# vitasoftAI/ImageRetrievalResearch

Hardware: AMD Instinct MI355X
Metric: images/sec embed + queries/sec top-k@100k-gallery, EffNet-B3a 224^2 (higher is better)
Workload: dtype bf16

## Files before the change

imageretrievalresearch_amd/csrc/rank.hip:

```cpp
#include "rank_common.h"
#include "../../include/mi355_retrieval.h"

#include <limits.h>
#include <stdlib.h>
#include <math.h>

namespace mi355 {

template <bool WRITE_ROWS>
__global__ __launch_bounds__(256) void k_row_norm(const float* __restrict__ in, float* __restrict__ out,
                                                  float* __restrict__ inv, i64 rows, int dim, float eps,
                                                  int vec) {
    const int lane = threadIdx.x & 63;
    const i64 row = (i64)blockIdx.x * 4 + (threadIdx.x >> 6);
    if (row >= rows) return;
    const float* x = in + row * dim;
    const float r = row_inv_norm(x, dim, eps, vec, lane);
    if (inv != nullptr && lane == 0) inv[row] = r;
    if (WRITE_ROWS) {
        float* y = out + row * dim;
        if (vec) {
            const f32x4* x4 = reinterpret_cast<const f32x4*>(x);
            f32x4* y4 = reinterpret_cast<f32x4*>(y);
            for (int i = lane; i < dim / 4; i += 64) {
// ... 128 lines not shown
        for (int i = 0; i < A_LOADS; ++i)
            *reinterpret_cast<f32x4*>(a + (r0 + RPP * i) * RK_LD + c4 * 4) = ra[i];
#pragma unroll
        for (int i = 0; i < B_LOADS; ++i)
            *reinterpret_cast<f32x4*>(b + (r0 + RPP * i) * RK_LD + c4 * 4) = rb[i];
    };

    const int nt = (D + RK_BK - 1) / RK_BK;
    load_tile(0);
    store_tile(0);
    __syncthreads();

    const int lr = lane & 31;
    const int lk = (lane >> 5) * 4;
    for (int t = 0; t < nt; ++t) {
        const int buf = t & 1;
        if (t + 1 < nt) load_tile((t + 1) * RK_BK);
        const float* a = As + buf * BM * RK_LD + (wm * MT * 32 + lr) * RK_LD + lk;
        const float* b = Bs + buf * RK_BN * RK_LD + (wn * 64 + lr) * RK_LD + lk;
#pragma unroll
        for (int t8 = 0; t8 < RK_BK / 8; ++t8) {
            f32x4 af[MT], bfr[2];
#pragma unroll
            for (int i = 0; i < MT; ++i) af[i] = *reinterpret_cast<const f32x4*>(a + i * 32 * RK_LD + t8 * 8);
#pragma unroll
            for (int j = 0; j < 2; ++j) bfr[j] = *reinterpret_cast<const f32x4*>(b + j * 32 * RK_LD + t8 * 8);
#pragma unroll
            for (int e = 0; e < 4; ++e)
#pragma unroll
                for (int i = 0; i < MT; ++i)
#pragma unroll
                    for (int j = 0; j < 2; ++j)
                        acc[i][j] = __builtin_amdgcn_mfma_f32_32x32x2f32(af[i][e], bfr[j][e], acc[i][j], 0, 0, 0);
        }
        if (t + 1 < nt) store_tile(buf ^ 1);
        __syncthreads();
    }

    epi.tile(acc, smem, ginv, TileCtx{Q, G, ntx, n0, m0});
}
template <int MT, int RK_BK, bool VEC, int FK>
__global__ __launch_bounds__(256) void k_cos_gemm(const float* __restrict__ Qn, const float* __restrict__ Gal,
                                                  const float* __restrict__ ginv, int Q, i64 G, int D, int x0, int ntx,
                                                  int xtiles, int ny, PlainEpi<FK> epi) {
    cos_gemm_f32_tile<MT, RK_BK, VEC>(Qn, Gal, ginv, Q, G, D, x0, ntx, xtiles, ny, epi);
}
template <int MT, int RK_BK, bool VEC, class Epi>
__global__ __launch_bounds__(256) void k_cos_gemm_epi(const float* __restrict__ Qn, const float* __restrict__ Gal,
                                                      const float* __restrict__ ginv, int Q, i64 G, int D, int x0, int ntx,
                                                      int xtiles, int ny, Epi epi) {
    cos_gemm_f32_tile<MT, RK_BK, VEC>(Qn, Gal, ginv, Q, G, D, x0, ntx, xtiles, ny, epi);
}

template <int MT, class Epi>
__device__ __forceinline__ void cos_gemm_split_tile(const bf16_t* __restrict__ Qs, const float* __restrict__ Gal,
                                                    const float* __restrict__ ginv, int Q, i64 G, int D, int x0, int ntx,
                                                    int n_steps, const float* __restrict__ zeros, int xtiles, int ny,
                                                    const Epi& epi) {
    constexpr int BM = 64 * MT;
    constexpr int BK = 16;
    constexpr int A_STAGE = (BM / 32) * 3 * 512;
    constexpr int A_PIECES = (BM / 32) * 3;
    constexpr int B_STAGE = RK_BN * BK;
    extern __shared__ __attribute__((aligned(16))) float smem[];
    bf16_t* As = reinterpret_cast<bf16_t*>(smem);
    constexpr int A_RING = MT == 1 ? 3 : 2;
    float* Bs = smem + (A_RING * A_STAGE * 2) / 4;

    const int tid = threadIdx.x, lane = tid & 63, wave = tid >> 6;
    const int wm = wave >> 1, wn = wave & 1;
    int bx, by;
    rank_tile_of((int)blockIdx.x, xtiles, ny, bx, by);
    const i64 n0 = (i64)(bx + x0) * RK_BN;
    const int m0 = by * BM;
    const int swave = __builtin_amdgcn_readfirstlane(wave);

    const float* b_row[2];
    int b_k[2];
    bool b_ok[2];
#pragma unroll
    for (int i = 0; i < 2; ++i) {
        const int r = (swave * 2 + i) * 16 + (lane >> 2);
        const int c = (lane & 3) ^ ((r >> 2) & 3);
        b_ok[i] = n0 + r < G;
        b_row[i] = Gal + (b_ok[i] ? (n0 + r) * D : 0);
        b_k[i] = c * 4;
    }
    auto dma_b = [&](int stage, int k0) {
#pragma unroll
        for (int i = 0; i < 2; ++i) {
            const bool ok = b_ok[i] && k0 + b_k[i] < D;
            glds16(reinterpret_cast<const bf16_t*>(ok ? b_row[i] + k0 + b_k[i] : zeros),
                   reinterpret_cast<bf16_t*>(Bs + stage * B_STAGE + (swave * 2 + i) * 256));
        }
    };
    const bf16_t* a_src = Qs + (size_t)(m0 / 32) * n_steps * 3 * 512 + lane * 8;
    const bf16_t* a_piece[(A_PIECES + 3) / 4];
#pragma unroll
    for (int i = 0; i < (A_PIECES + 3) / 4; ++i) {
        const int piece = (swave + 4 * i) % A_PIECES;
        a_piece[i] = a_src + ((size_t)((piece / 3) * n_steps) * 3 + piece % 3) * 512;
    }
    auto dma_a = [&](int buf, int t) {
#pragma unroll
        for (int i = 0; i < (A_PIECES + 3) / 4; ++i) {
            const int piece = swave + 4 * i;
            if (A_PIECES % 4 == 0 || i < A_PIECES / 4 || swave < A_PIECES % 4)
                glds16(a_piece[i] + (size_t)t * 3 * 512, As + buf * A_STAGE + piece * 512);
        }
    };

    f32x16 acc[MT][2];
#pragma unroll
    for (int i = 0; i < MT; ++i)
#pragma unroll
        for (int j = 0; j < 2; ++j)
#pragma unroll
            for (int e = 0; e < 16; ++e) acc[i][j][e] = 0.f;

    const int lr = lane & 31;
    int b_off[2][2];
#pragma unroll
    for (int j = 0; j < 2; ++j) {
        const int r = wn * 64 + j * 32 + lr, sw = (r >> 2) & 3, c0 = (lane >> 5) * 2;
        b_off[j][0] = r * BK + ((c0 ^ sw) << 2);
        b_off[j][1] = r * BK + (((c0 + 1) ^ sw) << 2);
    }
    auto compute = [&](int abuf, int bstage) {
        const bf16_t* a = As + abuf * A_STAGE + (wm * MT * 3) * 512 + lane * 8;
        const float* b = Bs + bstage * B_STAGE;
        bf16x8 af[MT][3];
        u32x4 bh[2], bm[2], bl[2];
        f32x4 v0[2], v1[2];
#pragma unroll
        for (int j = 0; j < 2; ++j) {
            v0[j] = *reinterpret_cast<const f32x4*>(b + b_off[j][0]);
            v1[j] = *reinterpret_cast<const f32x4*>(b + b_off[j][1]);
        }
#pragma unroll
        for (int i = 0; i < MT; ++i)
#pragma unroll
            for (int p = 0; p < 3; ++p) af[i][p] = *reinterpret_cast<const bf16x8*>(a + (i * 3 + p) * 512);
        split3(v0[0], v1[0], bh[0], bm[0], bl[0]);
        auto products = [&](int j) {
            const bf16x8 gh = *reinterpret_cast<const bf16x8*>(&bh[j]);
            const bf16x8 gm = *reinterpret_cast<const bf16x8*>(&bm[j]);
            const bf16x8 gl = *reinterpret_cast<const bf16x8*>(&bl[j]);
#pragma unroll
            for (int i = 0; i < MT; ++i) {
                acc[i][j] = __builtin_amdgcn_mfma_f32_32x32x16_bf16(af[i][2], gh, acc[i][j], 0, 0, 0);
                acc[i][j] = __builtin_amdgcn_mfma_f32_32x32x16_bf16(af[i][0], gl, acc[i][j], 0, 0, 0);
                acc[i][j] = __builtin_amdgcn_mfma_f32_32x32x16_bf16(af[i][1], gm, acc[i][j], 0, 0, 0);
                acc[i][j] = __builtin_amdgcn_mfma_f32_32x32x16_bf16(af[i][1], gh, acc[i][j], 0, 0, 0);
                acc[i][j] = __builtin_amdgcn_mfma_f32_32x32x16_bf16(af[i][0], gm, acc[i][j], 0, 0, 0);
                acc[i][j] = __builtin_amdgcn_mfma_f32_32x32x16_bf16(af[i][0], gh, acc[i][j], 0, 0, 0);
            }
        };
        split3(v0[1], v1[1], bh[1], bm[1], bl[1]);
        products(0);
#pragma unroll
        for (int g = 0; g < 6 * MT; ++g) {
            __builtin_amdgcn_sched_group_barrier(0x008, 1, 0);
            __builtin_amdgcn_sched_group_barrier(0x002, 4, 0);
        }
        products(1);
    };

    dma_a(0, 0);
    if (A_RING == 3 && n_steps > 1) dma_a(1, 1);
    dma_b(0, 0);
    dma_b(1, BK);
    __syncthreads();

    int bs_cur = 0, bs_far = 2;
    for (int t = 0; t < n_steps; ++t) {
        if constexpr (A_RING == 2) {
            if (t + 1 < n_steps) dma_a((t & 1) ^ 1, t + 1);
        } else {
            if (t + 2 < n_steps) dma_a(bs_far, t + 2);
        }
        __builtin_amdgcn_sched_barrier(0);
        dma_b(bs_far, (t + 2) * BK);
        __builtin_amdgcn_sched_barrier(0);
        compute(A_RING == 2 ? (t & 1) : bs_cur, bs_cur);
        if constexpr (A_RING == 2) {
            asm volatile("s_waitcnt vmcnt(2)" ::: "memory");
        } else {
            if (t + 2 >= n_steps) asm volatile("s_waitcnt vmcnt(2)" ::: "memory");
            else if (swave < A_PIECES % 4) asm volatile("s_waitcnt vmcnt(4)" ::: "memory");
            else asm volatile("s_waitcnt vmcnt(3)" ::: "memory");
        }
        asm volatile("s_waitcnt lgkmcnt(0)" ::: "memory");
        __builtin_amdgcn_s_barrier();
        asm volatile("" ::: "memory");
        bs_cur = bs_cur == 2 ? 0 : bs_cur + 1;
        bs_far = bs_far == 2 ? 0 : bs_far + 1;
    }
    __syncthreads();
    epi.tile(acc, smem, ginv, TileCtx{Q, G, ntx, n0, m0});
}
template <int MT, int FK>
__global__ __launch_bounds__(256, 3) void k_cos_gemm_split(const bf16_t* __restrict__ Qs, const float* __restrict__ Gal,
                                                           const float* __restrict__ ginv, int Q, i64 G, int D, int x0, int ntx,
                                                           int n_steps, const float* __restrict__ zeros, int xtiles, int ny,
                                                           PlainEpi<FK> epi) {
    cos_gemm_split_tile<MT>(Qs, Gal, ginv, Q, G, D, x0, ntx, n_steps, zeros, xtiles, ny, epi);
}
template <int MT, class Epi>
__global__ __launch_bounds__(256, 3) void k_cos_gemm_split_epi(const bf16_t* __restrict__ Qs, const float* __restrict__ Gal,
                                                               const float* __restrict__ ginv, int Q, i64 G, int D, int x0,
                                                               int ntx, int n_steps, const float* __restrict__ zeros, int xtiles,
                                                               int ny, Epi epi) {
    cos_gemm_split_tile<MT>(Qs, Gal, ginv, Q, G, D, x0, ntx, n_steps, zeros, xtiles, ny, epi);
}

template <int MT, int FK>
__global__ __launch_bounds__(256, 2) void k_cos_gemm_pre(const bf16_t* __restrict__ Qs, const bf16_t* __restrict__ Gs, int Q,
                                                         i64 G, int x0, int ntx, int n_steps, int xtiles, int ny,
                                                         SelectEpi<FK, false> epi) {
    constexpr int BM = 64 * MT;
    constexpr int A_PIECES = (BM / 32) * 3;
    constexpr int A_STAGE = A_PIECES * 512;
    constexpr int B_PIECES = (RK_BN / 32) * 3;
    constexpr int B_STAGE = B_PIECES * 512;
    constexpr int A_RING = MT == 1 ? 3 : 2;
    extern __shared__ __attribute__((aligned(16))) float smem[];
    bf16_t* As = reinterpret_cast<bf16_t*>(smem);
    bf16_t* Bs = As + A_RING * A_STAGE;

    const int tid = threadIdx.x, lane = tid & 63, wave = tid >> 6;
    const int wm = wave >> 1, wn = wave & 1;
    int bx, by;
    rank_tile_of((int)blockIdx.x, xtiles, ny, bx, by);
    const i64 n0 = (i64)(bx + x0) * RK_BN;
    const int m0 = by * BM;
    const int swave = __builtin_amdgcn_readfirstlane(wave);

    const bf16_t* a_src = Qs + (size_t)(m0 / 32) * n_steps * 3 * 512 + lane * 8;
    const bf16_t* b_src = Gs + (size_t)(n0 / 32) * n_steps * 3 * 512 + lane * 8;
    const bf16_t* a_piece[(A_PIECES + 3) / 4];
    const bf16_t* b_piece[3];
#pragma unroll
    for (int i = 0; i < (A_PIECES + 3) / 4; ++i) {
        const int piece = (swave + 4 * i) % A_PIECES;
        a_piece[i] = a_src + ((size_t)((piece / 3) * n_steps) * 3 + piece % 3) * 512;
    }
#pragma unroll
    for (int i = 0; i < 3; ++i) {
        const int piece = swave + 4 * i;
        b_piece[i] = b_src + ((size_t)((piece / 3) * n_steps) * 3 + piece % 3) * 512;
    }
    auto dma_a = [&](int buf, int t) {
#pragma unroll
        for (int i = 0; i < (A_PIECES + 3) / 4; ++i) {
            const int piece = swave + 4 * i;
            if (A_PIECES % 4 == 0 || i < A_PIECES / 4 || swave < A_PIECES % 4)
                glds16(a_piece[i] + (size_t)t * 3 * 512, As + buf * A_STAGE + piece * 512);
        }
    };
    auto dma_b = [&](int stage, int t) {
        const int tt = t < n_steps ? t : n_steps - 1;
#pragma unroll
        for (int i = 0; i < 3; ++i) glds16(b_piece[i] + (size_t)tt * 3 * 512, Bs + stage * B_STAGE + (swave + 4 * i) * 512);
    };

    f32x16 acc[MT][2];
// ... 481 lines not shown
}

int kernel_slots(const void* fn, size_t lds, int* cache, int* slots_out) {
    int dev = 0;
    MI355_CHECK_HIP(hipGetDevice(&dev));
    MI355_REQUIRE(dev >= 0 && dev < MI355_MAX_DEVICES, "rank: device ordinal %d out of range", dev);
    if (!cache[dev]) {
        MI355_CHECK_HIP(hipFuncSetAttribute(fn, hipFuncAttributeMaxDynamicSharedMemorySize, (int)lds));
        int per_cu = 0, cus = 0;
        MI355_CHECK_HIP(hipOccupancyMaxActiveBlocksPerMultiprocessor(&per_cu, fn, 256, lds));
        MI355_CHECK_HIP(hipDeviceGetAttribute(&cus, hipDeviceAttributeMultiprocessorCount, dev));
        cache[dev] = (per_cu > 0 ? per_cu : 1) * (cus > 0 ? cus : 1);
    }
    *slots_out = cache[dev];
    return OK;
}

int whole_round_tiles(int ntx, int ny, int slots) {
    if ((long)ntx * ny > slots && ((long)ntx * ny) % slots != 0) return (int)(((long)ntx * ny / slots) * slots / ny);
    return ntx;
}

static thread_local int g_round_slots = 0;
static thread_local int g_last_tiles[5] = {0, 0, 0, 0, 0};
int round_slots(int device_slots) { return g_round_slots > 0 ? g_round_slots : device_slots; }
void set_last_tiles(int slots, int ny, int main_tiles, int tail_tiles, int tail_ny) {
    g_last_tiles[0] = slots; g_last_tiles[1] = ny; g_last_tiles[2] = main_tiles; g_last_tiles[3] = tail_tiles;
    g_last_tiles[4] = tail_ny;
}

template <bool VEC>
struct F32Gemm {
    template <int MT> static constexpr int BK = MT == 2 ? 16 : 32;
    template <int MT> static constexpr size_t stage_bytes() { return (size_t)2 * (64 * MT + RK_BN) * (BK<MT> + 4) * sizeof(float); }
    template <int MT, class Epi> static constexpr auto kernel() {
        if constexpr (plain_fk<Epi> >= 0) return &k_cos_gemm<MT, BK<MT>, VEC, plain_fk<Epi>>;
        else return &k_cos_gemm_epi<MT, BK<MT>, VEC, Epi>;
    }
    template <int MT, class Epi>
    static void launch(dim3 grid, size_t lds, hipStream_t st, const TileArgs& a, const Epi& epi, int x0, int ntx, int xtiles, int ny) {
        hipLaunchKernelGGL((kernel<MT, Epi>()), grid, dim3(256), lds, st, (const float*)a.qry, (const float*)a.gal, a.ginv, a.Q, a.G,
                           a.D, x0, ntx, xtiles, ny, epi);
    }
};

struct SplitGemm {
    template <int MT> static constexpr size_t stage_bytes() {
        return (size_t)(MT == 1 ? 3 : 2) * (64 * MT / 32) * 3 * 1024 + (size_t)3 * RK_BN * 16 * sizeof(float);
    }
    template <int MT, class Epi> static constexpr auto kernel() {
        if constexpr (plain_fk<Epi> >= 0) return &k_cos_gemm_split<MT, plain_fk<Epi>>;
        else return &k_cos_gemm_split_epi<MT, Epi>;
    }
    template <int MT, class Epi>
    static void launch(dim3 grid, size_t lds, hipStream_t st, const TileArgs& a, const Epi& epi, int x0, int ntx, int xtiles, int ny) {
        const bf16_t* qs = (const bf16_t*)a.qry;
        const int n_steps = cdiv(a.D, 16);
        const float* zeros = reinterpret_cast<const float*>(qs + (size_t)cdiv(a.Q, 128) * 4 * n_steps * 3 * 512);
        hipLaunchKernelGGL((kernel<MT, Epi>()), grid, dim3(256), lds, st, qs, (const float*)a.gal, a.ginv, a.Q, a.G, a.D, x0, ntx,
                           n_steps, zeros, xtiles, ny, epi);
    }
};

struct PreparedGemm {
    template <int MT> static constexpr size_t stage_bytes() {
        return (size_t)(MT == 1 ? 3 : 2) * (64 * MT / 32) * 3 * 1024 + (size_t)3 * (RK_BN / 32) * 3 * 1024;
    }
    template <int MT, class Epi> static constexpr auto kernel() {
        static_assert(plain_fk<Epi> > 0, "the prepared gallery has fused unfiltered kernels only");
        return &k_cos_gemm_pre<MT, plain_fk<Epi>>;
    }
    template <int MT, class Epi>
    static void launch(dim3 grid, size_t lds, hipStream_t st, const TileArgs& a, const Epi& epi, int x0, int ntx, int xtiles, int ny) {
        hipLaunchKernelGGL((kernel<MT, Epi>()), grid, dim3(256), lds, st, (const bf16_t*)a.qry, (const bf16_t*)a.gal, a.Q, a.G, x0,
                           ntx, cdiv(a.D, 16), xtiles, ny, epi);
    }
};

static bool rank_exact_f32() {
    const char* e = getenv("MI355_RANK_EXACT_F32");
    return e && e[0] && e[0] != '0';
}

template <class Epi>
static int cos_gemm(const float* qn, bf16_t* qs, const float* gal, const float* ginv, i64 Q, i64 G, int D, const Epi& epi,
                    hipStream_t st) {
    const bool vec = vec_ok(qn, D) && vec_ok(gal, D);
    constexpr int fused_bit = is_select<Epi> ? MI355_RANK_PATH_FUSED : 0;
    if constexpr (std::is_same_v<Epi, SlabEpi>) {
        if (Q <= 4 && (size_t)Q * D * sizeof(float) <= 60 * 1024) {
            set_rank_path(MI355_RANK_PATH_GEMV);
            const size_t lds = (size_t)Q * D * sizeof(float);
            const unsigned blocks = (unsigned)(cdiv(G, 4) < 4096 ? cdiv(G, 4) : 4096);
#define GEMV_LAUNCH(NQ) hipLaunchKernelGGL((k_cos_gemv<NQ>), dim3(blocks), dim3(256), lds, st, qn, gal, ginv, epi.S, G, D, (int)vec)
            if (Q == 1) GEMV_LAUNCH(1); else if (Q == 2) GEMV_LAUNCH(2); else if (Q == 3) GEMV_LAUNCH(3); else GEMV_LAUNCH(4);
#undef GEMV_LAUNCH
            MI355_LAUNCH_CHECK();
            return OK;
        }
    }
    TileArgs a{qn, gal, ginv, (int)Q, G, D};
    if (qs && vec_ok(gal, D) && !rank_exact_f32()) {
        if (int e = split_rows(qn, Q, D, qs, st)) return e;
        set_rank_path(MI355_RANK_PATH_SPLIT | fused_bit);
        a.qry = qs;
        return cos_gemm_tiles<SplitGemm>(a, epi, st);
    }
    set_rank_path(MI355_RANK_PATH_EXACT_F32 | fused_bit);
    return vec ? cos_gemm_tiles<F32Gemm<true>>(a, epi, st) : cos_gemm_tiles<F32Gemm<false>>(a, epi, st);
}

int normalize_search(const float* queries, i64 Q, const float* gallery, i64 G, int dim, float eps, const RankWs& w,
                     hipStream_t st) {
    const int vq = vec_ok(queries, dim) && vec_ok(w.qn, dim);
    RoctxRange range("rank/normalize");
// ... 499 lines not shown
```

imageretrievalresearch_amd/csrc/rank_common.h:

```cpp
#pragma once
#include "common.h"
#include "../../include/mi355_retrieval.h"

#include <limits.h>
#include <math.h>
#include <type_traits>

namespace mi355 {

typedef float f32x4 __attribute__((ext_vector_type(4)));
typedef float f32x16 __attribute__((ext_vector_type(16)));
typedef long long i64;

constexpr float NEG_INF = -INFINITY;
constexpr i64 IDX_PAD = LLONG_MAX;
constexpr i64 NO_CAND_IDX = (i64)1 << 62;

constexpr int IDX32_PAD = INT_MAX;

__device__ __forceinline__ unsigned score_key(float x) {
    const unsigned u = __float_as_uint(x + 0.0f);
    if ((u & 0x7fffffffu) > 0x7f800000u) return 0xffffffffu;
    return (u & 0x80000000u) ? ~u : (u | 0x80000000u);
}
// ... 58 lines not shown
struct SlabEpi {
    float* S;
    template <size_t STAGE> static constexpr size_t lds_bytes() { return STAGE; }
    template <int MT>
    __device__ __forceinline__ void tile(f32x16 (&acc)[MT][2], float*, const float* __restrict__ ginv, const TileCtx& t) const {
        const int Q = t.Q, m0 = t.m0;
        const i64 G = t.G, n0 = t.n0;
        const int tid = threadIdx.x, lane = tid & 63, wave = tid >> 6;
        const int wm = wave >> 1, wn = wave & 1, lr = lane & 31;
#pragma unroll
        for (int j = 0; j < 2; ++j) {
            const i64 col = n0 + wn * 64 + j * 32 + lr;
            if (col >= G) continue;
            const float gs = ginv ? ginv[col] : 1.0f;
#pragma unroll
            for (int i = 0; i < MT; ++i) {
#pragma unroll
                for (int r = 0; r < 16; ++r) {
                    const int row = m0 + wm * MT * 32 + i * 32 + (r & 3) + 8 * (r >> 2) + 4 * (lane >> 5);
                    if (row < Q) S[(i64)row * G + col] = acc[i][j][r] * gs;
                }
            }
        }
    }
};

constexpr size_t EPI_TILE_BYTES = (size_t)64 * (RK_BN + 4) * sizeof(float);

template <int FK, bool FILT>
struct SelectEpi {
    int k;
    float* cand_val;
    int* cand_idx;
    RankFilter flt;
    template <size_t STAGE> static constexpr size_t lds_bytes() {
        static_assert(!FILT || STAGE >= EPI_TILE_BYTES + FILT_LABELS_BYTES, "the filtered epilogue would grow the GEMM's LDS");
        return EPI_TILE_BYTES > STAGE ? EPI_TILE_BYTES : STAGE;
    }
    template <int MT>
    __device__ __forceinline__ void tile(f32x16 (&acc)[MT][2], float* smem, const float* __restrict__ ginv, const TileCtx& t) const {
        static_assert(FK > 0, "the fused selection keeps at least one candidate");
        const int Q = t.Q, ntx = t.ntx, m0 = t.m0;
        const i64 G = t.G, n0 = t.n0;
        constexpr int BM = 64 * MT;
        const int tid = threadIdx.x, lane = tid & 63, wave = tid >> 6;
        const int wm = wave >> 1, wn = wave & 1, lr = lane & 31;
        constexpr int CLD = RK_BN + 4;
        float* Ct = smem;
        const i64 ncol = (G - n0 < RK_BN) ? G - n0 : RK_BN;
        i64* glab = reinterpret_cast<i64*>(smem + 64 * CLD);
        if constexpr (FILT) {
            if (tid < RK_BN) glab[tid + (tid >> 5)] = (flt.mode != MI355_LABEL_ANY && tid < ncol) ? flt.glab[n0 + tid] : 0;
        }
#pragma unroll 1
        for (int h = 0; h < BM / 64; ++h) {
            if ((wm * MT * 32) / 64 == h) {
#pragma unroll
                for (int j = 0; j < 2; ++j) {
                    const i64 col = n0 + wn * 64 + j * 32 + lr;
                    const float gs = (ginv && col < G) ? ginv[col] : 1.0f;
#pragma unroll
                    for (int i = 0; i < MT; ++i)
#pragma unroll
                        for (int r = 0; r < 16; ++r) {
                            const int row = (wm * MT * 32) % 64 + i * 32 + (r & 3) + 8 * (r >> 2) + 4 * (lane >> 5);
                            Ct[row * CLD + wn * 64 + j * 32 + lr] = acc[i][j][r] * gs;
                        }
                }
            }
            __syncthreads();
            {
                const int lrow = tid >> 2, part = tid & 3;
                unsigned kv[FK];
                int ki[FK];
#pragma unroll
                for (int i = 0; i < FK; ++i) { kv[i] = 0u; ki[i] = IDX32_PAD; }
                auto insert = [&](unsigned key, int id) {
                    bool g[FK];
#pragma unroll
                    for (int i = 0; i < FK; ++i) g[i] = key > kv[i];
#pragma unroll
                    for (int i = FK - 1; i > 0; --i) {
                        kv[i] = g[i] ? (g[i - 1] ? kv[i - 1] : key) : kv[i];
                        ki[i] = g[i] ? (g[i - 1] ? ki[i - 1] : id) : ki[i];
                    }
                    kv[0] = g[0] ? key : kv[0];
                    ki[0] = g[0] ? id : ki[0];
                };
                const float* rowp = Ct + lrow * CLD + part * 32;
                i64 fq_lab = 0, fq_ex = -1;
                if constexpr (FILT) {
                    if (m0 + h * 64 + lrow < Q) query_filter(flt, m0 + h * 64 + lrow, fq_lab, fq_ex);
                }
#pragma unroll 2
                for (int c4i = 0; c4i < 8; ++c4i) {
                    const f32x4 v4 = *reinterpret_cast<const f32x4*>(rowp + c4i * 4);
                    const float vv[4] = {v4.x, v4.y, v4.z, v4.w};
#pragma unroll
                    for (int e = 0; e < 4; ++e) {
                        const int c = part * 32 + c4i * 4 + e;
                        unsigned key = score_key(vv[e]);
                        if (c >= ncol) key = 0u;
                        if constexpr (FILT) {
                            if (!eligible(flt.mode, fq_lab, glab[c + part], fq_ex, n0 + c)) key = 0u;
                        }
                        if (__any(key > kv[FK - 1])) insert(key, (int)n0 + c);
                    }
                }
#pragma unroll
                for (int src = 1; src < 4; ++src) {
#pragma unroll
                    for (int i = 0; i < FK; ++i) {
                        const unsigned ok = (unsigned)__shfl(kv[i], (lane & ~3) + src, 64);
                        const int oi = __shfl(ki[i], (lane & ~3) + src, 64);
                        if (part == 0) insert(ok, oi);
                    }
                }
                const int qrow = m0 + h * 64 + lrow;
                if (part == 0 && qrow < Q) {
                    const size_t o = ((size_t)qrow * ntx + (size_t)(n0 / RK_BN)) * k;
#pragma unroll
                    for (int i = 0; i < FK; ++i)
                        if (i < k) { cand_val[o + i] = ki[i] == IDX32_PAD ? NEG_INF : key_score(kv[i]); cand_idx[o + i] = ki[i]; }
                }
            }
            __syncthreads();
        }
    }
};

constexpr int ROC_MAX_T = MI355_ROC_MAX_THRESHOLDS;
constexpr int ROC_SUB_T = 1024;
constexpr int ROC_BIN_WORDS = ROC_MAX_T + 4;
constexpr size_t ROC_EPI_BYTES = (size_t)ROC_MAX_T * sizeof(float) + (size_t)ROC_BIN_WORDS * sizeof(unsigned) +
                                 (size_t)3 * RK_BN * sizeof(i64);

__host__ __device__ __forceinline__ float roc_ceil_f32(double t) {
    float f = (float)t;
    if ((double)f < t) f = nextafterf(f, INFINITY);
    return f;
}

struct RocArgs {
    const i64* qlab;
    const i64* glab;
    const i64* excl;
    i64 idx_offset;
    const double* thr;
    unsigned long long* hist;
    int T;
    int top;
    int uniform;
    float scale;
    template <size_t STAGE> static constexpr size_t lds_bytes() { return ROC_EPI_BYTES > STAGE ? ROC_EPI_BYTES : STAGE; }
    template <int MT>
    __device__ __forceinline__ void tile(f32x16 (&acc)[MT][2], float* smem, const float* __restrict__ ginv, const TileCtx& t) const;
};

template <class V>
__device__ __forceinline__ int roc_bin(V s, const V* tab, const RocArgs& a) {
    if (a.uniform) {
        if (!(s >= tab[0])) return 0;
        const V x = (s - tab[0]) * (V)a.scale;
        int g = x < (V)(a.T - 1) ? (int)x + 1 : a.T;
        while (g < a.T && s >= tab[g]) ++g;
        while (s < tab[g - 1]) --g;
        return g;
    }
    int b = 0;
    for (int step = a.top; step > 0; step >>= 1)
        if (b + step <= a.T && tab[b + step - 1] <= s) b += step;
// ... 337 lines not shown
        }
    } else {
        if constexpr (VEC) {
            const f32x4* x4 = reinterpret_cast<const f32x4*>(x);
            for (int i = lane; i < ld / 4; i += 64) {
                f16x4_t h = {(_Float16)0.f, (_Float16)0.f, (_Float16)0.f, (_Float16)0.f};
                if (i < nu) {
                    const f32x4 v = x4[i];
                    h = (f16x4_t){scaled_f16(v.x, r), scaled_f16(v.y, r), scaled_f16(v.z, r), scaled_f16(v.w, r)};
                }
                reinterpret_cast<f16x4_t*>(y)[i] = h;
            }
        } else {
            for (int i = lane; i < ld; i += 64) y[i] = i < dim ? scaled_f16(x[i], r) : (_Float16)0.f;
        }
    }
}

static inline int vec_ok(const void* p, int dim) { return (dim % 4 == 0) && (((uintptr_t)p & 15) == 0); }

constexpr int SMALL_K = 8;
constexpr int LARGE_K = 1024;

size_t topk_ws_bytes(i64 Q, i64 G, int k);
int topk_select(const float* vals, const i64* idxs, i64 Q, i64 rowlen, i64 in_stride, int k, i64 idx_offset, float* out_val,
                i64* out_idx, void* ws, size_t ws_bytes, hipStream_t st, const int* idxs32 = nullptr,
                const RankFilter* filt = nullptr);
RankFilter filter_from(const RankFilter& f, i64 q0);
int make_filter(const mi355_rank_filter* f, i64 idx_offset, const char* who, RankFilter* out);
void set_rank_path(int path);
bool fused_select(i64 Q, i64 G, int k);
i64 query_block(i64 Q, i64 G, int k);
int kernel_slots(const void* fn, size_t lds, int* cache, int* slots_out);
int whole_round_tiles(int ntx, int ny, int slots);
int round_slots(int device_slots);
void set_last_tiles(int slots, int ny, int main_tiles, int tail_tiles, int tail_ny);

template <int FK> using PlainEpi = std::conditional_t<FK == 0, SlabEpi, SelectEpi<(FK > 0 ? FK : 1), false>>;
template <class Epi> constexpr int plain_fk = -1;
template <> inline constexpr int plain_fk<SlabEpi> = 0;
template <int FK> constexpr int plain_fk<SelectEpi<FK, false>> = FK;
template <class Epi> constexpr bool is_select = false;
template <int FK, bool FILT> constexpr bool is_select<SelectEpi<FK, FILT>> = true;

struct TileArgs {
    const void* qry;
    const void* gal;
    const float* ginv;
    int Q;
    i64 G;
    int D;
};

template <class F, int MT, class Epi>
int launch_tiles(const TileArgs& a, const Epi& epi, hipStream_t st, int x0 = 0, bool tail = false) {
    constexpr size_t lds = Epi::template lds_bytes<F::template stage_bytes<MT>()>();
    static int cache[MI355_MAX_DEVICES] = {0};
    int slots = 0;
    if (int e = kernel_slots((const void*)F::template kernel<MT, Epi>(), lds, cache, &slots)) return e;
    const int ntx = cdiv(a.G, RK_BN), ny = cdiv(a.Q, 64 * MT);
    if (!tail) slots = round_slots(slots);
    const int x1 = MT == 2 ? whole_round_tiles(ntx, ny, slots) : ntx;
    if (!tail) set_last_tiles(slots, ny, x1, ntx - x1, x1 < ntx ? cdiv(a.Q, 64) : 0);
    if (x1 > x0) {
        F::template launch<MT, Epi>(dim3((unsigned)(x1 - x0) * (unsigned)ny), lds, st, a, epi, x0, ntx, x1 - x0, ny);
        MI355_LAUNCH_CHECK();
    }
    if constexpr (MT == 2) {
        if (x1 < ntx) return launch_tiles<F, 1, Epi>(a, epi, st, x1, true);
    }
    return OK;
}
template <class F, class Epi>
int cos_gemm_tiles(const TileArgs& a, const Epi& epi, hipStream_t st) {
    return a.Q > 64 ? launch_tiles<F, 2, Epi>(a, epi, st) : launch_tiles<F, 1, Epi>(a, epi, st);
}

template <bool FILT, class Fn>
int with_select_epi(int k, float* cand_val, int* cand_idx, const RankFilter& f, Fn&& fn) {
    if (k <= 1) return fn(SelectEpi<1, FILT>{k, cand_val, cand_idx, f});
    if (k <= 2) return fn(SelectEpi<2, FILT>{k, cand_val, cand_idx, f});
    if (k <= 4) return fn(SelectEpi<4, FILT>{k, cand_val, cand_idx, f});
    return fn(SelectEpi<8, FILT>{k, cand_val, cand_idx, f});
}

int roc_check_thresholds(const double* thr, int T, const char* who, RocArgs* a);
int roc_check_pairs(const int64_t* query_labels, const int64_t* gallery_labels, const int64_t* exclude, int64_t idx_offset,
                    const double* thresholds_dev, int64_t* hist, const char* who, RocArgs* a);
RocArgs roc_from(const RocArgs& a, i64 q0);
i64 roc_query_block(i64 Q, i64 G);

struct RankWs {
    float* qn; void* qs; float* ginv; float* S; float* cand_val; int* cand_idx; void* topk; size_t topk_bytes; size_t total;
};
RankWs carve(void* ws, i64 Q, i64 G, int D, int k, size_t (*planes_bytes)(i64, int), bool need_ginv, bool need_S = true);
int normalize_search(const float* queries, i64 Q, const float* gallery, i64 G, int dim, float eps, const RankWs& w,
                     hipStream_t st);

template <class Fn>
int with_topk_epi(const RankWs& w, int k, const RankFilter* f, Fn&& fn) {
    if (!w.cand_val) return fn(SlabEpi{w.S});
    if (f) return with_select_epi<true>(k, w.cand_val, w.cand_idx, *f, fn);
    return with_select_epi<false>(k, w.cand_val, w.cand_idx, RankFilter{}, fn);
}

template <class Score>
int search_blocks(const float* queries, const float* gallery_to_norm, i64 Q, i64 G, int dim, int k, float eps, i64 idx_offset,
                  const RankFilter* filt, float* out_val, i64* out_idx, const RankWs& w, hipStream_t st, const char* slab_range,
                  Score&& score) {
    if (int e = normalize_search(queries, Q, gallery_to_norm, G, dim, eps, w, st)) return e;
    const bool fused = fused_select(Q, G, k);
    const i64 qb = query_block(Q, G, k), rowlen = fused ? cdiv(G, RK_BN) * (i64)k : G;
    for (i64 q0 = 0; q0 < Q; q0 += qb) {
// ... 69 lines not shown
```

Baseline: 62480.

## Add deep-ring tail GEMM kernel and threshold-prefiltered top-k epilogue

Adds a separate tail kernel for the 64-query remainder tiles. It uses a deeper (default six-stage) LDS ring with fragment double-buffering, so loads for later k-steps are in flight while the current step runs. It is launched only when the remaining tiles fit in one wave of slots. The select epilogue now unrolls the row-half loop, builds a per-lane running top-FK threshold with fmed3 and inserts only columns at or above that threshold, and merges partial lists with DPP moves instead of shuffles. The cost is more LDS per block for the tail, a more complex epilogue, and possible register pressure.

```diff
diff --git a/imageretrievalresearch_amd/csrc/rank.hip b/imageretrievalresearch_amd/csrc/rank.hip
--- a/imageretrievalresearch_amd/csrc/rank.hip
+++ b/imageretrievalresearch_amd/csrc/rank.hip
@@ -204,7 +204,7 @@
     cos_gemm_f32_tile<MT, RK_BK, VEC>(Qn, Gal, ginv, Q, G, D, x0, ntx, xtiles, ny, epi);
 }
 
-template <int MT, class Epi>
+template <int MT, int RING, class Epi>
 __device__ __forceinline__ void cos_gemm_split_tile(const bf16_t* __restrict__ Qs, const float* __restrict__ Gal,
                                                     const float* __restrict__ ginv, int Q, i64 G, int D, int x0, int ntx,
                                                     int n_steps, const float* __restrict__ zeros, int xtiles, int ny,
@@ -216,7 +216,8 @@
     constexpr int B_STAGE = RK_BN * BK;
     extern __shared__ __attribute__((aligned(16))) float smem[];
     bf16_t* As = reinterpret_cast<bf16_t*>(smem);
-    constexpr int A_RING = MT == 1 ? 3 : 2;
+    static_assert(RING == 0 || (MT == 1 && RING >= 3), "the deep ring is the 64-query tail's");
+    constexpr int A_RING = RING ? RING : MT == 1 ? 3 : 2;
     float* Bs = smem + (A_RING * A_STAGE * 2) / 4;
 
     const int tid = threadIdx.x, lane = tid & 63, wave = tid >> 6;
@@ -257,8 +258,10 @@
 #pragma unroll
         for (int i = 0; i < (A_PIECES + 3) / 4; ++i) {
             const int piece = swave + 4 * i;
-            if (A_PIECES % 4 == 0 || i < A_PIECES / 4 || swave < A_PIECES % 4)
-                glds16(a_piece[i] + (size_t)t * 3 * 512, As + buf * A_STAGE + piece * 512);
+            if (A_PIECES % 4 == 0 || i < A_PIECES / 4 || swave < A_PIECES % 4) {
+                const bf16_t* src = RING && t >= n_steps ? reinterpret_cast<const bf16_t*>(zeros) : a_piece[i] + (size_t)t * 3 * 512;
+                glds16(src, As + buf * A_STAGE + piece * 512);
+            }
         }
     };
 
@@ -318,35 +321,125 @@
         products(1);
     };
 
-    dma_a(0, 0);
-    if (A_RING == 3 && n_steps > 1) dma_a(1, 1);
-    dma_b(0, 0);
-    dma_b(1, BK);
-    __syncthreads();
-
-    int bs_cur = 0, bs_far = 2;
-    for (int t = 0; t < n_steps; ++t) {
-        if constexpr (A_RING == 2) {
-            if (t + 1 < n_steps) dma_a((t & 1) ^ 1, t + 1);
-        } else {
-            if (t + 2 < n_steps) dma_a(bs_far, t + 2);
-        }
-        __builtin_amdgcn_sched_barrier(0);
-        dma_b(bs_far, (t + 2) * BK);
-        __builtin_amdgcn_sched_barrier(0);
-        compute(A_RING == 2 ? (t & 1) : bs_cur, bs_cur);
-        if constexpr (A_RING == 2) {
-            asm volatile("s_waitcnt vmcnt(2)" ::: "memory");
-        } else {
-            if (t + 2 >= n_steps) asm volatile("s_waitcnt vmcnt(2)" ::: "memory");
-            else if (swave < A_PIECES % 4) asm volatile("s_waitcnt vmcnt(4)" ::: "memory");
-            else asm volatile("s_waitcnt vmcnt(3)" ::: "memory");
-        }
-        asm volatile("s_waitcnt lgkmcnt(0)" ::: "memory");
+    if constexpr (RING == 0) {
+        dma_a(0, 0);
+        if (A_RING == 3 && n_steps > 1) dma_a(1, 1);
+        dma_b(0, 0);
+        dma_b(1, BK);
+        __syncthreads();
+
+        int bs_cur = 0, bs_far = 2;
+        for (int t = 0; t < n_steps; ++t) {
+            if constexpr (A_RING == 2) {
+                if (t + 1 < n_steps) dma_a((t & 1) ^ 1, t + 1);
+            } else {
+                if (t + 2 < n_steps) dma_a(bs_far, t + 2);
+            }
+            __builtin_amdgcn_sched_barrier(0);
+            dma_b(bs_far, (t + 2) * BK);
+            __builtin_amdgcn_sched_barrier(0);
+            compute(A_RING == 2 ? (t & 1) : bs_cur, bs_cur);
+            if constexpr (A_RING == 2) {
+                asm volatile("s_waitcnt vmcnt(2)" ::: "memory");
+            } else {
+                if (t + 2 >= n_steps) asm volatile("s_waitcnt vmcnt(2)" ::: "memory");
+                else if (swave < A_PIECES % 4) asm volatile("s_waitcnt vmcnt(4)" ::: "memory");
+                else asm volatile("s_waitcnt vmcnt(3)" ::: "memory");
+            }
+            asm volatile("s_waitcnt lgkmcnt(0)" ::: "memory");
+            __builtin_amdgcn_s_barrier();
+            asm volatile("" ::: "memory");
+            bs_cur = bs_cur == 2 ? 0 : bs_cur + 1;
+            bs_far = bs_far == 2 ? 0 : bs_far + 1;
+        }
+    } else {
+        static_assert(RING >= 4, "k-steps t + 1 and t + 2 land while t runs");
+        constexpr int AHEAD = RING - 1;
+#pragma unroll 1
+        for (int s = 0; s < AHEAD; ++s) {
+            dma_a(s, s);
+            __builtin_amdgcn_sched_barrier(0);
+            dma_b(s, s * BK);
+            __builtin_amdgcn_sched_barrier(0);
+        }
+        auto wait_landed = [&]() {
+            if (swave < A_PIECES % 4) asm volatile("s_waitcnt vmcnt(%0)" ::"n"((RING - 3) * 4) : "memory");
+            else asm volatile("s_waitcnt vmcnt(%0)" ::"n"((RING - 3) * 3) : "memory");
+        };
+        struct Frags {
+            bf16x8 a[3];
+            u32x4 h0, m0, l0;
+            f32x4 x0, x1;
+        };
+        auto six = [&](int j, const Frags& f, const u32x4& h, const u32x4& m, const u32x4& l) __attribute__((always_inline)) {
+            const bf16x8 gh = *reinterpret_cast<const bf16x8*>(&h);
+            const bf16x8 gm = *reinterpret_cast<const bf16x8*>(&m);
+            const bf16x8 gl = *reinterpret_cast<const bf16x8*>(&l);
+            acc[0][j] = __builtin_amdgcn_mfma_f32_32x32x16_bf16(f.a[2], gh, acc[0][j], 0, 0, 0);
+            acc[0][j] = __builtin_amdgcn_mfma_f32_32x32x16_bf16(f.a[0], gl, acc[0][j], 0, 0, 0);
+            acc[0][j] = __builtin_amdgcn_mfma_f32_32x32x16_bf16(f.a[1], gm, acc[0][j], 0, 0, 0);
+            acc[0][j] = __builtin_amdgcn_mfma_f32_32x32x16_bf16(f.a[1], gh, acc[0][j], 0, 0, 0);
+            acc[0][j] = __builtin_amdgcn_mfma_f32_32x32x16_bf16(f.a[0], gm, acc[0][j], 0, 0, 0);
+            acc[0][j] = __builtin_amdgcn_mfma_f32_32x32x16_bf16(f.a[0], gh, acc[0][j], 0, 0, 0);
+        };
+        auto fetch = [&](int slot, Frags& f, f32x4& y0, f32x4& y1) __attribute__((always_inline)) {
+            const bf16_t* a = As + slot * A_STAGE + (wm * 3) * 512 + lane * 8;
+            const float* b = Bs + slot * B_STAGE;
+            y0 = *reinterpret_cast<const f32x4*>(b + b_off[0][0]);
+            y1 = *reinterpret_cast<const f32x4*>(b + b_off[0][1]);
+            f.x0 = *reinterpret_cast<const f32x4*>(b + b_off[1][0]);
+            f.x1 = *reinterpret_cast<const f32x4*>(b + b_off[1][1]);
+#pragma unroll
+            for (int p = 0; p < 3; ++p) f.a[p] = *reinterpret_cast<const bf16x8*>(a + p * 512);
+        };
+        int cur = 0, far = AHEAD;
+        auto step = [&](int t, Frags& now, Frags& next) __attribute__((always_inline)) {
+            dma_a(far, t + AHEAD);
+            __builtin_amdgcn_sched_barrier(0);
+            dma_b(far, (t + AHEAD) * BK);
+            __builtin_amdgcn_sched_barrier(0);
+            f32x4 y0, y1;
+            fetch(cur == RING - 1 ? 0 : cur + 1, next, y0, y1);
+            u32x4 h1, m1, l1;
+            split3(now.x0, now.x1, h1, m1, l1);
+            six(0, now, now.h0, now.m0, now.l0);
+#pragma unroll
+            for (int g = 0; g < 6; ++g) {
+                __builtin_amdgcn_sched_group_barrier(0x008, 1, 0);
+                __builtin_amdgcn_sched_group_barrier(0x002, 6, 0);
+            }
+            __builtin_amdgcn_sched_barrier(0);
+            split3(y0, y1, next.h0, next.m0, next.l0);
+            six(1, now, h1, m1, l1);
+#pragma unroll
+            for (int g = 0; g < 6; ++g) {
+                __builtin_amdgcn_sched_group_barrier(0x008, 1, 0);
+                __builtin_amdgcn_sched_group_barrier(0x002, 6, 0);
+            }
+            asm volatile("" : "+v"(next.h0), "+v"(next.m0), "+v"(next.l0));
+            __builtin_amdgcn_sched_barrier(0);
+            wait_landed();
+            asm volatile("s_waitcnt lgkmcnt(0)" ::: "memory");
+            __builtin_amdgcn_s_barrier();
+            asm volatile("" ::: "memory");
+            cur = cur == RING - 1 ? 0 : cur + 1;
+            far = far == RING - 1 ? 0 : far + 1;
+        };
+        wait_landed();
         __builtin_amdgcn_s_barrier();
         asm volatile("" ::: "memory");
-        bs_cur = bs_cur == 2 ? 0 : bs_cur + 1;
-        bs_far = bs_far == 2 ? 0 : bs_far + 1;
+        Frags even, odd;
+        {
+            f32x4 y0, y1;
+            fetch(0, even, y0, y1);
+            split3(y0, y1, even.h0, even.m0, even.l0);
+        }
+        int t = 0;
+        for (; t + 1 < n_steps; t += 2) {
+            step(t, even, odd);
+            step(t + 1, odd, even);
+        }
+        if (t < n_steps) step(t, even, odd);
     }
     __syncthreads();
     epi.tile(acc, smem, ginv, TileCtx{Q, G, ntx, n0, m0});
@@ -356,14 +449,32 @@
                                                            const float* __restrict__ ginv, int Q, i64 G, int D, int x0, int ntx,
                                                            int n_steps, const float* __restrict__ zeros, int xtiles, int ny,
                                                            PlainEpi<FK> epi) {
-    cos_gemm_split_tile<MT>(Qs, Gal, ginv, Q, G, D, x0, ntx, n_steps, zeros, xtiles, ny, epi);
+    cos_gemm_split_tile<MT, 0>(Qs, Gal, ginv, Q, G, D, x0, ntx, n_steps, zeros, xtiles, ny, epi);
 }
 template <int MT, class Epi>
 __global__ __launch_bounds__(256, 3) void k_cos_gemm_split_epi(const bf16_t* __restrict__ Qs, const float* __restrict__ Gal,
                                                                const float* __restrict__ ginv, int Q, i64 G, int D, int x0,
                                                                int ntx, int n_steps, const float* __restrict__ zeros, int xtiles,
                                                                int ny, Epi epi) {
-    cos_gemm_split_tile<MT>(Qs, Gal, ginv, Q, G, D, x0, ntx, n_steps, zeros, xtiles, ny, epi);
+    cos_gemm_split_tile<MT, 0>(Qs, Gal, ginv, Q, G, D, x0, ntx, n_steps, zeros, xtiles, ny, epi);
+}
+#ifndef MI355_TAIL_RING
+#define MI355_TAIL_RING 6
+#endif
+constexpr int TAIL_RING = MI355_TAIL_RING;
+template <int FK>
+__global__ __launch_bounds__(256) void k_cos_gemm_split_tail(const bf16_t* __restrict__ Qs, const float* __restrict__ Gal,
+                                                             const float* __restrict__ ginv, int Q, i64 G, int D, int x0, int ntx,
+                                                             int n_steps, const float* __restrict__ zeros, int xtiles, int ny,
+                                                             PlainEpi<FK> epi) {
+    cos_gemm_split_tile<1, TAIL_RING>(Qs, Gal, ginv, Q, G, D, x0, ntx, n_steps, zeros, xtiles, ny, epi);
+}
+template <class Epi>
+__global__ __launch_bounds__(256) void k_cos_gemm_split_tail_epi(const bf16_t* __restrict__ Qs, const float* __restrict__ Gal,
+                                                                 const float* __restrict__ ginv, int Q, i64 G, int D, int x0,
+                                                                 int ntx, int n_steps, const float* __restrict__ zeros, int xtiles,
+                                                                 int ny, Epi epi) {
+    cos_gemm_split_tile<1, TAIL_RING>(Qs, Gal, ginv, Q, G, D, x0, ntx, n_steps, zeros, xtiles, ny, epi);
 }
 
 template <int MT, int FK>
@@ -951,15 +1062,36 @@
         if constexpr (plain_fk<Epi> >= 0) return &k_cos_gemm_split<MT, plain_fk<Epi>>;
         else return &k_cos_gemm_split_epi<MT, Epi>;
     }
-    template <int MT, class Epi>
-    static void launch(dim3 grid, size_t lds, hipStream_t st, const TileArgs& a, const Epi& epi, int x0, int ntx, int xtiles, int ny) {
+    template <class K, class Epi>
+    static void launch_kernel(K kern, dim3 grid, size_t lds, hipStream_t st, const TileArgs& a, const Epi& epi, int x0, int ntx,
+                              int xtiles, int ny) {
         const bf16_t* qs = (const bf16_t*)a.qry;
         const int n_steps = cdiv(a.D, 16);
         const float* zeros = reinterpret_cast<const float*>(qs + (size_t)cdiv(a.Q, 128) * 4 * n_steps * 3 * 512);
-        hipLaunchKernelGGL((kernel<MT, Epi>()), grid, dim3(256), lds, st, qs, (const float*)a.gal, a.ginv, a.Q, a.G, a.D, x0, ntx,
-                           n_steps, zeros, xtiles, ny, epi);
+        hipLaunchKernelGGL(kern, grid, dim3(256), lds, st, qs, (const float*)a.gal, a.ginv, a.Q, a.G, a.D, x0, ntx, n_steps, zeros,
+                           xtiles, ny, epi);
+    }
+    template <int MT, class Epi>
+    static void launch(dim3 grid, size_t lds, hipStream_t st, const TileArgs& a, const Epi& epi, int x0, int ntx, int xtiles, int ny) {
+        launch_kernel(kernel<MT, Epi>(), grid, lds, st, a, epi, x0, ntx, xtiles, ny);
     }
 };
+
+struct SplitTailGemm {
+    template <int MT> static constexpr size_t stage_bytes() {
+        static_assert(MT == 1, "the tail launch runs 64-query tiles");
+        return (size_t)TAIL_RING * (2 * 3 * 1024 + RK_BN * 16 * sizeof(float));
+    }
+    template <int MT, class Epi> static constexpr auto kernel() {
+        if constexpr (plain_fk<Epi> >= 0) return &k_cos_gemm_split_tail<plain_fk<Epi>>;
+        else return &k_cos_gemm_split_tail_epi<Epi>;
+    }
+    template <int MT, class Epi>
+    static void launch(dim3 grid, size_t lds, hipStream_t st, const TileArgs& a, const Epi& epi, int x0, int ntx, int xtiles, int ny) {
+        SplitGemm::launch_kernel(kernel<MT, Epi>(), grid, lds, st, a, epi, x0, ntx, xtiles, ny);
+    }
+};
+template <> struct TailFamily<SplitGemm> { using type = SplitTailGemm; };
 
 struct PreparedGemm {
     template <int MT> static constexpr size_t stage_bytes() {
diff --git a/imageretrievalresearch_amd/csrc/rank_common.h b/imageretrievalresearch_amd/csrc/rank_common.h
--- a/imageretrievalresearch_amd/csrc/rank_common.h
+++ b/imageretrievalresearch_amd/csrc/rank_common.h
@@ -134,20 +134,17 @@
         if constexpr (FILT) {
             if (tid < RK_BN) glab[tid + (tid >> 5)] = (flt.mode != MI355_LABEL_ANY && tid < ncol) ? flt.glab[n0 + tid] : 0;
         }
-#pragma unroll 1
+        const bool whole = ncol == RK_BN;
+#pragma unroll
         for (int h = 0; h < BM / 64; ++h) {
-            if ((wm * MT * 32) / 64 == h) {
-#pragma unroll
-                for (int j = 0; j < 2; ++j) {
-                    const i64 col = n0 + wn * 64 + j * 32 + lr;
-                    const float gs = (ginv && col < G) ? ginv[col] : 1.0f;
-#pragma unroll
-                    for (int i = 0; i < MT; ++i)
-#pragma unroll
-                        for (int r = 0; r < 16; ++r) {
-                            const int row = (wm * MT * 32) % 64 + i * 32 + (r & 3) + 8 * (r >> 2) + 4 * (lane >> 5);
-                            Ct[row * CLD + wn * 64 + j * 32 + lr] = acc[i][j][r] * gs;
-                        }
+#pragma unroll
+            for (int j = 0; j < 2; ++j) {
+                const i64 col = n0 + wn * 64 + j * 32 + lr;
+                const float gs = (ginv && col < G) ? ginv[col] : 1.0f;
+#pragma unroll
+                for (int r = 0; r < 16; ++r) {
+                    const int row = wm * 32 + (r & 3) + 8 * (r >> 2) + 4 * (lane >> 5);
+                    Ct[row * CLD + wn * 64 + j * 32 + lr] = acc[h][j][r] * gs;
                 }
             }
             __syncthreads();
@@ -170,35 +167,78 @@
                     ki[0] = g[0] ? id : ki[0];
                 };
                 const float* rowp = Ct + lrow * CLD + part * 32;
-                i64 fq_lab = 0, fq_ex = -1;
-                if constexpr (FILT) {
-                    if (m0 + h * 64 + lrow < Q) query_filter(flt, m0 + h * 64 + lrow, fq_lab, fq_ex);
-                }
+                const int qrow = m0 + (lrow >> 5) * (MT * 32) + h * 32 + (lrow & 31);
+                bool full_scan = FILT || !whole;
+                if (!FILT && whole) {
+                    float tv[FK];
+#pragma unroll
+                    for (int i = 0; i < FK; ++i) tv[i] = NEG_INF;
+                    bool nan = false;
+#pragma unroll
+                    for (int c4i = 0; c4i < 8; ++c4i) {
+                        const f32x4 v4 = *reinterpret_cast<const f32x4*>(rowp + c4i * 4);
+                        const float vv[4] = {v4.x, v4.y, v4.z, v4.w};
+#pragma unroll
+                        for (int e = 0; e < 4; ++e) {
+                            nan |= vv[e] != vv[e];
+#pragma unroll
+                            for (int i = FK - 1; i > 0; --i) tv[i] = __builtin_amdgcn_fmed3f(tv[i - 1], tv[i], vv[e]);
+                            tv[0] = __builtin_amdgcn_fmed3f(tv[0], vv[e], INFINITY);
+                        }
+                    }
+                    full_scan = __any(nan);
+                    if (!full_scan) {
+                        const float thr = tv[FK - 1];
+                        unsigned mask = 0u;
+#pragma unroll
+                        for (int c4i = 0; c4i < 8; ++c4i) {
+                            const f32x4 v4 = *reinterpret_cast<const f32x4*>(rowp + c4i * 4);
+                            const float vv[4] = {v4.x, v4.y, v4.z, v4.w};
+#pragma unroll
+                            for (int e = 0; e < 4; ++e) mask = (mask << 1) | (vv[e] >= thr ? 1u : 0u);
+                        }
+                        while (__any(mask != 0u)) {
+                            if (mask != 0u) {
+                                const int c = __clz((int)mask);
+                                mask &= ~(0x80000000u >> c);
+                                insert(score_key(rowp[c]), (int)n0 + part * 32 + c);
+                            }
+                        }
+                    }
+                }
+                if (full_scan) {
+                    i64 fq_lab = 0, fq_ex = -1;
+                    if constexpr (FILT) {
+                        if (qrow < Q) query_filter(flt, qrow, fq_lab, fq_ex);
+                    }
 #pragma unroll 2
-                for (int c4i = 0; c4i < 8; ++c4i) {
-                    const f32x4 v4 = *reinterpret_cast<const f32x4*>(rowp + c4i * 4);
-                    const float vv[4] = {v4.x, v4.y, v4.z, v4.w};
-#pragma unroll
-                    for (int e = 0; e < 4; ++e) {
-                        const int c = part * 32 + c4i * 4 + e;
-                        unsigned key = score_key(vv[e]);
-                        if (c >= ncol) key = 0u;
-                        if constexpr (FILT) {
-                            if (!eligible(flt.mode, fq_lab, glab[c + part], fq_ex, n0 + c)) key = 0u;
+                    for (int c4i = 0; c4i < 8; ++c4i) {
+                        const f32x4 v4 = *reinterpret_cast<const f32x4*>(rowp + c4i * 4);
+                        const float vv[4] = {v4.x, v4.y, v4.z, v4.w};
+#pragma unroll
+                        for (int e = 0; e < 4; ++e) {
+                            const int c = part * 32 + c4i * 4 + e;
+                            unsigned key = score_key(vv[e]);
+                            if (c >= ncol) key = 0u;
+                            if constexpr (FILT) {
+                                if (!eligible(flt.mode, fq_lab, glab[c + part], fq_ex, n0 + c)) key = 0u;
+                            }
+                            if (__any(key > kv[FK - 1])) insert(key, (int)n0 + c);
                         }
-                        if (__any(key > kv[FK - 1])) insert(key, (int)n0 + c);
                     }
                 }
 #pragma unroll
-                for (int src = 1; src < 4; ++src) {
-#pragma unroll
-                    for (int i = 0; i < FK; ++i) {
-                        const unsigned ok = (unsigned)__shfl(kv[i], (lane & ~3) + src, 64);
-                        const int oi = __shfl(ki[i], (lane & ~3) + src, 64);
-                        if (part == 0) insert(ok, oi);
-                    }
-                }
-                const int qrow = m0 + h * 64 + lrow;
+                for (int i = 0; i < FK; ++i) {
+                    const unsigned ok = (unsigned)__builtin_amdgcn_mov_dpp((int)kv[i], 0xB1, 0xf, 0xf, true);
+                    const int oi = __builtin_amdgcn_mov_dpp(ki[i], 0xB1, 0xf, 0xf, true);
+                    if ((part & 1) == 0) insert(ok, oi);
+                }
+#pragma unroll
+                for (int i = 0; i < FK; ++i) {
+                    const unsigned ok = (unsigned)__builtin_amdgcn_mov_dpp((int)kv[i], 0x4E, 0xf, 0xf, true);
+                    const int oi = __builtin_amdgcn_mov_dpp(ki[i], 0x4E, 0xf, 0xf, true);
+                    if (part == 0) insert(ok, oi);
+                }
                 if (part == 0 && qrow < Q) {
                     const size_t o = ((size_t)qrow * ntx + (size_t)(n0 / RK_BN)) * k;
 #pragma unroll
@@ -642,6 +682,7 @@
     int D;
 };
 
+template <class F> struct TailFamily { using type = F; };
 template <class F, int MT, class Epi>
 int launch_tiles(const TileArgs& a, const Epi& epi, hipStream_t st, int x0 = 0, bool tail = false) {
     constexpr size_t lds = Epi::template lds_bytes<F::template stage_bytes<MT>()>();
@@ -649,6 +690,20 @@
     int slots = 0;
     if (int e = kernel_slots((const void*)F::template kernel<MT, Epi>(), lds, cache, &slots)) return e;
     const int ntx = cdiv(a.G, RK_BN), ny = cdiv(a.Q, 64 * MT);
+    if constexpr (MT == 1 && !std::is_same_v<typename TailFamily<F>::type, F>) {
+        if (tail) {
+            using T = typename TailFamily<F>::type;
+            constexpr size_t tail_lds = Epi::template lds_bytes<T::template stage_bytes<1>()>();
+            static int tail_cache[MI355_MAX_DEVICES] = {0};
+            int tail_slots = 0;
+            if (int e = kernel_slots((const void*)T::template kernel<1, Epi>(), tail_lds, tail_cache, &tail_slots)) return e;
+            if ((long)(ntx - x0) * ny <= tail_slots) {
+                T::template launch<1, Epi>(dim3((unsigned)(ntx - x0) * (unsigned)ny), tail_lds, st, a, epi, x0, ntx, ntx - x0, ny);
+                MI355_LAUNCH_CHECK();
+                return OK;
+            }
+        }
+    }
     if (!tail) slots = round_slots(slots);
     const int x1 = MT == 2 ? whole_round_tiles(ntx, ny, slots) : ntx;
     if (!tail) set_last_tiles(slots, ny, x1, ntx - x1, x1 < ntx ? cdiv(a.Q, 64) : 0);
```

Measured after the change: 63070, median of 6. Within noise of the previous version (+0.9%).
